# naturerobots/mesh_navigation

Hardware: AMD Instinct MI355X
Metric: plans/sec (Dijkstra makePlan device path incl. computeVectorMap, 1M-vertex mesh) (higher is better)
Workload: dtype f32

## Files before the change

### include/mnav.h

```cpp
#ifndef MNAV_H
#define MNAV_H

#include <stdint.h>

#ifdef __cplusplus
extern "C" {
#endif

#define MNAV_SUCCESS 0u
#define MNAV_CANCELED 51u
#define MNAV_INVALID_START 52u
#define MNAV_INVALID_GOAL 53u
#define MNAV_NO_PATH_FOUND 54u
#define MNAV_INTERNAL_ERROR 60u
#define MNAV_NONE 0xFFFFFFFFu

typedef struct mnav_ctx mnav_ctx;

typedef struct mnav_stats {
  uint32_t steps;
  uint32_t launches;
  uint32_t bands;
  uint32_t armed;
  float goal_dist;
// ... 309 lines not shown
uint64_t mnav_device_bytes(const mnav_ctx* ctx);

int mnav_shard_begin(mnav_ctx* ctx, uint32_t seed_vertex, uint32_t target_vertex, double goal_dist_offset, double cost_limit);
int mnav_shard_set_goal_tie(mnav_ctx* ctx, uint32_t tie_id);
int mnav_shard_rounds(mnav_ctx* ctx, uint32_t rounds, float* iface_buf_dev);
int mnav_shard_apply(mnav_ctx* ctx, const float* iface_buf_dev, float* local_min_out, float* target_dist_out);
int mnav_shard_finalize(mnav_ctx* ctx, float* dist_buf_dev, uint32_t* pred_buf_dev);
int mnav_shard_rounds_async(mnav_ctx* ctx, uint32_t rounds, float* iface_buf_dev, void* caller_stream);
int mnav_shard_apply_async(mnav_ctx* ctx, const float* iface_buf_dev, float* ctl_dev, void* caller_stream);

void mnav_cancel(mnav_ctx* ctx);

int mnav_get_stats(const mnav_ctx* ctx, mnav_stats* out);
int mnav_get_timing(const mnav_ctx* ctx, mnav_stats* out);
int mnav_tb_finalize_stats(mnav_ctx* ctx, uint64_t* skipped_pairs, uint64_t* reset_pairs, uint32_t* filled_at_start);
int mnav_set_band_width(mnav_ctx* ctx, float delta);
int mnav_set_dijkstra_engine(mnav_ctx* ctx, int engine);
int mnav_set_option(mnav_ctx* ctx, const char* name, double value);
double mnav_get_option(const mnav_ctx* ctx, const char* name);
int mnav_set_resident_outputs(mnav_ctx* ctx, int on);
int mnav_download_output(mnav_ctx* ctx, uint32_t slot, int what, void* host_out);
int mnav_vector_at(mnav_ctx* ctx, uint32_t slot, const uint32_t vs[3], const float bary[3], float out[3]);
int mnav_backtrack_cvp_batch(mnav_ctx* ctx, uint32_t n, const float* seed_pos, const uint32_t* seed_faces, const float* target_pos,
                             const uint32_t* target_faces, double step_width, int32_t inflation_layer, uint32_t cap,
                             float* positions_out, uint32_t* faces_out, uint32_t* n_out, int32_t* status_out);
int mnav_backtrack_cvp(mnav_ctx* ctx, const float seed_pos[3], uint32_t seed_face, const float target_pos[3], uint32_t target_face,
                       double step_width, int32_t inflation_layer, uint32_t cap, float* positions_out, uint32_t* faces_out,
                       uint32_t* n_out);
const void* mnav_device_output(const mnav_ctx* ctx, uint32_t slot, int what);
uint64_t mnav_algorithmic_bytes(const mnav_ctx* ctx);
// ... 7 lines not shown
```

### mesh_navigation_amd/capi.py

```python
from __future__ import annotations

import ctypes as C
import os
import sys
import time
import weakref
from dataclasses import dataclass

import numpy as np

from . import build as _build

NONE = 0xFFFFFFFF
SUCCESS, CANCELED, INVALID_START, INVALID_GOAL, NO_PATH_FOUND, INTERNAL_ERROR = 0, 51, 52, 53, 54, 60
SCHEDULE_NONE, SCHEDULE_COMMITTED, SCHEDULE_NO_SLOT, SCHEDULE_OPEN = 0, 1, 2, 3
SCHEDULE_SEED_FREE = 1
BEYOND_FIELD = 70
WALK_NO_FACE = -3

SYMBOLS = [
    "mnav_create", "mnav_destroy", "mnav_last_error", "mnav_set_face_circulation", "mnav_upload_mesh", "mnav_upload_costs",
    "mnav_compute_edge_weights", "mnav_combine_costs", "mnav_plan_dijkstra", "mnav_plan_cvp", "mnav_plan_dijkstra_batch", "mnav_plan_cvp_batch",
    "mnav_cancel", "mnav_get_stats", "mnav_get_timing", "mnav_tb_finalize_stats", "mnav_set_band_width", "mnav_set_dijkstra_engine", "mnav_device_output",
    "mnav_algorithmic_bytes", "mnav_shard_setup", "mnav_shard_setup_partition", "mnav_shard_walk", "mnav_device_bytes", "mnav_shard_info", "mnav_shard_begin", "mnav_shard_rounds", "mnav_shard_apply", "mnav_shard_rounds_async", "mnav_shard_apply_async",
    "mnav_shard_finalize", "mnav_update_costs", "mnav_update_edge_weights", "mnav_download_costs", "mnav_set_resident_outputs", "mnav_download_output",
    "mnav_vector_at", "mnav_backtrack_cvp", "mnav_backtrack_cvp_batch", "mnav_layer_upload", "mnav_layer_steepness", "mnav_layer_inflation", "mnav_layer_download",
    "mnav_combine_layers", "mnav_layer_stats", "mnav_layer_download_vectors", "mnav_combine_layers_update",
    "mnav_layer_obstacle", "mnav_obstacle_stats",
    "mnav_layer_height_diff", "mnav_layer_roughness", "mnav_layer_ridge", "mnav_neighbourhood_stats",
    "mnav_layer_border", "mnav_layer_clearance", "mnav_clearance_download", "mnav_clearance_stats",
    "mnav_locate", "mnav_locate_stats", "mnav_plan_dijkstra_batch_at", "mnav_plan_cvp_batch_at",
    "mnav_follow_batch", "mnav_follow_stats", "mnav_follow_rollout", "mnav_rollout_stats", "mnav_fleet_rollout", "mnav_fleet_rollout_stats",
    "mnav_fleet_rollout_yield", "mnav_fleet_yield_stats", "mnav_fleet_rollout_rings", "mnav_fleet_ring_stats",
    "mnav_map_configure", "mnav_map_compute", "mnav_map_layer_changed", "mnav_map_update_layer", "mnav_map_obstacle", "mnav_map_stats",
    "mnav_replan_dijkstra_batch", "mnav_replan_plans", "mnav_replan_stats", "mnav_replan_dijkstra_each", "mnav_replan_each_stats",
    "mnav_replan_warm_stats",
    "mnav_fleet_paths", "mnav_fleet_walks", "mnav_fleet_stats",
    "mnav_upload_face_normals", "mnav_fleet_plans", "mnav_fleet_walk_plans",
# ... 247 lines not shown
    L.mnav_replan_each_stats.argtypes = ([vp] + [C.POINTER(u32)] * 3 + [vp, vp, vp] + [C.POINTER(C.c_uint64)] * 2 + [C.POINTER(u32)] * 2
                                         + [C.POINTER(C.c_int32), vp])
    L.mnav_replan_warm_stats.restype = C.c_int
    L.mnav_replan_warm_stats.argtypes = [vp] + [C.POINTER(u32)] * 3 + [C.POINTER(C.c_uint64)] * 2 + [vp] + [C.POINTER(u32)] * 2
    L.mnav_replan_plans.restype = u32
    L.mnav_replan_plans.argtypes = [vp]
    L.mnav_replan_stats.restype = C.c_int
    L.mnav_replan_stats.argtypes = [vp, C.POINTER(u32), C.POINTER(u32), vp] + [C.POINTER(C.c_uint64)] * 2 + [C.POINTER(u32)] * 2 + [C.POINTER(C.c_float)] * 4
    L.mnav_cancel.argtypes = [vp]
    L.mnav_get_stats.restype = C.c_int
    L.mnav_get_stats.argtypes = [vp, C.POINTER(Stats)]
    L.mnav_get_timing.restype = C.c_int
    L.mnav_get_timing.argtypes = [vp, C.POINTER(Stats)]
    L.mnav_tb_finalize_stats.restype = C.c_int
    L.mnav_tb_finalize_stats.argtypes = [vp, C.POINTER(C.c_uint64), C.POINTER(C.c_uint64), C.POINTER(u32)]
    L.mnav_set_band_width.restype = C.c_int
    L.mnav_set_band_width.argtypes = [vp, C.c_float]
    L.mnav_set_dijkstra_engine.restype = C.c_int
    L.mnav_set_dijkstra_engine.argtypes = [vp, C.c_int]
    L.mnav_shard_set_goal_tie.restype = C.c_int
    L.mnav_shard_set_goal_tie.argtypes = [vp, u32]
    L.mnav_set_option.restype = C.c_int
    L.mnav_set_option.argtypes = [vp, C.c_char_p, C.c_double]
    L.mnav_get_option.restype = C.c_double
    L.mnav_get_option.argtypes = [vp, C.c_char_p]
    L.mnav_device_output.restype = vp
    L.mnav_device_output.argtypes = [vp, u32, C.c_int]
    L.mnav_set_resident_outputs.restype = C.c_int
    L.mnav_set_resident_outputs.argtypes = [vp, C.c_int]
    L.mnav_download_output.restype = C.c_int
# ... 563 lines not shown
            raise RuntimeError(f"mnav_shard_finalize failed ({rc}): {self._err()}")

    def stats(self) -> dict:
        s = Stats()
        self._L.mnav_get_stats(self._h, C.byref(s))
        d = s.as_dict()
        d["algorithmic_bytes"] = int(self._L.mnav_algorithmic_bytes(self._h))
        return d

    def tb_finalize_stats(self) -> dict:
        sk, rs, fl = C.c_uint64(0), C.c_uint64(0), C.c_uint32(0)
        if self._L.mnav_tb_finalize_stats(self._h, C.byref(sk), C.byref(rs), C.byref(fl)) != 0:
            raise RuntimeError(f"mnav_tb_finalize_stats failed: {self._err()}")
        return dict(skipped_pairs=int(sk.value), reset_pairs=int(rs.value), filled_at_start=bool(fl.value))

    def last_engine(self) -> str:
        e = int(self._L.mnav_last_engine(self._h))
        if e >= 256:
            ran = (["k_tile_round (tile rounds)"] if e & 128 else []) + ([_warm_name(1 if e & 1024 else 0)] if e & 512 else [])
            ran += [_engine_name(e & 127)] if (e & 127) != 127 else []
            return " + ".join(ran) if ran else "none (every plan kept)"
        if e in (5, 21) and self.replan_warm_stats()["live"]:
            return _warm_name(1 if e == 21 else 0)
        return _engine_name(e)

    def timing(self) -> dict:
        s = Stats()
        self._L.mnav_get_timing(self._h, C.byref(s))
        return s.as_dict()

# ... 648 lines not shown
```

### mesh_navigation_amd/csrc/mnav.hip

```cpp
#include <hip/hip_runtime.h>

#include <algorithm>
#include <array>
#include <atomic>
#include <chrono>
#include <cmath>
#include <cstdio>
#include <cstdlib>
#include <cstring>
#include <functional>
#include <map>
#include <string>
#include <vector>
#include <unordered_map>
#include <unistd.h>

#include "../../include/mnav.h"
#include "mnav_buf.h"
#include "mnav_build.h"
#include "mnav_eval.h"
#include "mnav_options.h"
#include "mnav_resident.h"

using namespace mnav;
// ... 1732 lines not shown
    if (hipSetDevice(ctx->device) != hipSuccess) { ctx->err = "hipSetDevice failed"; return -1; }
    const uint32_t nblk = (S.fin_np + 63u) / 64u;
    HIPCHK(hipMemsetAsync(S.fin_cnt, 0, 16, ctx->stream));
    hipLaunchKernelGGL(k_tb_fin_count, dim3(std::min<uint32_t>(((size_t)S.ntiles * nblk + kBlock - 1) / kBlock, 1024u)), dim3(kBlock), 0, ctx->stream,
                       S.umap.get(), S.uskip.get(), S.ntiles, nblk, S.umap_stride, S.fin_cnt.get());
    HIPCHK(hipGetLastError());
    HIPCHK(hipMemcpyAsync(cnt, S.fin_cnt, 16, hipMemcpyDeviceToHost, ctx->stream));
    HIPCHK(hipStreamSynchronize(ctx->stream));
  }
  if (skipped_pairs) *skipped_pairs = cnt[1];
  if (reset_pairs) *reset_pairs = (S.fin_stats && S.fin_reset) ? (uint64_t)S.ntiles * S.fin_np - cnt[0] : 0u;
  if (filled_at_start) *filled_at_start = S.filled_at_start ? 1u : 0u;
  return 0;
}

int mnav_get_timing(const mnav_ctx* ctx, mnav_stats* out)
{
  if (!ctx || !out) return -1;
  *out = ctx->stats;
  if (ctx->tb.count_pending) out->settled = 0;
  return 0;
}

int mnav_set_band_width(mnav_ctx* ctx, float delta)
{
  if (!ctx) return -1;
  ctx->delta_user = delta > 0.f ? delta : 0.f;
  return 0;
}

// ... 237 lines not shown
```

### mesh_navigation_amd/csrc/mnav_options.h

```cpp
#pragma once

#define MNAV_OPTION_LIST(X)                                                                                                              \
  X(verbose)                                                              \
  X(trace)                                                                                       \
  X(no_graph)             \
  X(debug_chunk)          \
  X(dijkstra_engine)                                 \
  X(blocks_per_plan)                                                                                 \
  X(tile_blocks)                                                                                    \
  X(cvp_wide)                                        \
  X(wide_waves)                                                                                      \
  X(cvp_groups)                          \
  X(max_steps) X(max_wall_s)                                                                                                             \
  X(cvp_verify)                                                                     \
  X(key_walk_max) X(descend_walk_max)                                                               \
  X(tile_size)                                                                                   \
  X(lazy_paths)                                                                                      \
  X(tile_band) X(rounds_band_mult)                                                                                                       \
  X(tb_tile)                                                       \
  X(tb_no_prefill) X(tb_band_mult) X(tb_waves_per_cu)                                                                                    \
  X(tb_kernel)            \
  X(tb_sched_lds)         \
  X(tb_fin_keep)          \
  X(tb_fin_cnt8)          \
  X(async_wg_per_cu) X(async_wg_per_plan) X(async_max_s)                                                                          \
  X(async_band_mult)                              \
  X(async_max_batch)                                           \
  X(async_ring_cap)             \
  X(nbhd_lds_cap)         \
  X(replan_log_cap)                                          \
  X(replan_fresh_below)   \
  X(replan_each_fresh_share)  \
  X(replan_repair_engine)  \
  X(replan_warm_min_plans)  \
  X(fleet_scratch_mb)     \
  X(dispatch_max_mb)      \
  X(dispatch_max_rounds)  \
// ... 52 lines not shown
```

### mesh_navigation_amd/csrc/mnav_tb.h

```cpp
#pragma once

#include "mnav_tb_build.h"

namespace {

namespace tb {

#define MNAV_CONST __attribute__((address_space(4)))
typedef uint32_t u32x16 __attribute__((ext_vector_type(16)));
typedef const MNAV_CONST u32x16* cblk8_t;
typedef __attribute__((address_space(3))) uint32_t* lds_u32_t;
enum { kTwSoff = 0, kTwSl = 1, kTwNv = 2, kTwNh = 3, kTwSweepOff = 4, kTwSweepChunks = 5, kTwPreOff = 6, kTwPreChunks = 7,
       kTwPostOff = 8, kTwPostChunks = 9, kTwExpOff = 10, kTwExpN = 11 };
static_assert(offsetof(TbTile, exp_n) == 4 * kTwExpN && offsetof(TbTile, sweep_off) == 4 * kTwSweepOff, "TbTile layout");

struct Ctl {
  uint32_t n_cand[2];
  uint32_t n_items, next_item;
  uint32_t err;
  uint32_t iters;
  unsigned long long acts;
  unsigned long long sweeps;
  unsigned long long items;
  unsigned long long wakes;
// ... 1 lines not shown

struct Args {
  const TbTile* tiles; const uint32_t* stream; const TbExp* exps;
  float* D; uint32_t* pend; uint32_t NP, ntiles;
  uint16_t* bucket; uint32_t* bcnt; uint2* items; Ctl* ctl;
  uint32_t* marr[2];
  uint32_t* mcarry;
  float* thr; float* bnd;
  const uint32_t* seed; const uint32_t* target;
  const uint2* vaddr; const uint32_t* vert_tile;
  double offset; float band;
  uint8_t* pflag; uint32_t nblk;
  unsigned long long* wstat; uint32_t wstat_slots;
  uint32_t item_plans;
  uint32_t sched_lds, min_copies;
};

__device__ __forceinline__ size_t slot_addr(const uint2 va, uint32_t NP, uint32_t p)
{
  return (size_t)va.x * NP + (size_t)p * (va.y >> 8) + (va.y & 255u);
}

__device__ __forceinline__ uint32_t ldsr(uint32_t off) { return *(lds_u32_t)(uintptr_t)off; }
__device__ __forceinline__ void ldsw(uint32_t off, uint32_t v) { *(lds_u32_t)(uintptr_t)off = v; }
typedef __attribute__((address_space(3))) u32x4* lds_u32x4_t;
__device__ __forceinline__ u32x4 ldsr4(uint32_t off) { return *(lds_u32x4_t)(uintptr_t)off; }

__device__ __forceinline__ uint32_t rfl(uint32_t x) { return (uint32_t)__builtin_amdgcn_readfirstlane((int)x); }

}
// ... 802 lines not shown
```

### mesh_navigation_amd/csrc/mnav_tb_host.h

```cpp
#pragma once

void tb_free_batch(mnav_ctx* ctx)
{
  TbState& S = ctx->tb;
  if (S.fill_stream) (void)hipStreamSynchronize(S.fill_stream);
  static_cast<TbBatch&>(S) = TbBatch{};
  S.count_pending = false; ctx->tb_args_valid = false;
  ctx->res.batch_state_freed();
}

void tb_free(mnav_ctx* ctx)
{
  tb_free_batch(ctx);
  static_cast<TbTables&>(ctx->tb) = TbTables{};
}

int tb_build(mnav_ctx* ctx)
{
  TbState& S = ctx->tb;
  if (S.built) return 0;
  if (opt_set(ctx->opt.tb_tile)) S.T = opt_u32(ctx->opt.tb_tile, S.T);
  if (S.T != 64 && S.T != 96 && S.T != 120 && S.T != 128) S.T = 120;
  HostTopology t;
  t.V = ctx->V; t.E = ctx->E; t.F = ctx->F;
// ... 254 lines not shown
  HIPCHK(hipMemsetAsync(ctx->d_mismatch, 0, 4, ctx->stream));
  if (!ctx->lazy_paths && tb_fields_upload(ctx, n, in, offset)) return -1;
  tb::Args A{};
  A.tiles = S.d_tiles; A.stream = S.d_stream; A.exps = S.d_exps; A.D = S.D; A.pend = S.pend; A.pflag = S.pflag; A.nblk = (n + 63u) / 64u; A.NP = n; A.ntiles = S.ntiles;
  A.bucket = S.bucket; A.bcnt = S.bcnt; A.items = S.items; A.ctl = S.ctl; A.wstat = S.wstat; A.wstat_slots = kTbStatSlots;
  A.marr[0] = S.marr[0]; A.marr[1] = S.marr[1]; A.mcarry = S.mcarry;
  A.thr = S.thr; A.bnd = S.bnd; A.seed = S.seed; A.target = S.target; A.vaddr = S.d_vaddr; A.vert_tile = S.d_vert_tile;
  A.offset = offset;
  const bool v_fits = S.T == 120 && S.max_nh <= kTbvGhostRows;
  const double density = (double)n / std::sqrt((double)std::max(S.ntiles, 1u));
  S.kernel = (v_fits && density >= 8.0) ? 1 : 0;
  if (opt_set(ctx->opt.tb_kernel)) S.kernel = (opt_u32(ctx->opt.tb_kernel, 0u) == 1u && v_fits) ? 1 : 0;
  A.item_plans = S.kernel == 1 ? 64u : kTbItemPlans;
  A.sched_lds = (tb_sched_lds_fits(n) && !(opt_set(ctx->opt.tb_sched_lds) && !opt_on(ctx->opt.tb_sched_lds))) ? 1u : 0u;
  A.min_copies = A.sched_lds ? kTbMinCopiesLds : kTbMinCopies;
  {
    const float band_mult = (S.kernel == 1 && density < 40.0) ? 4.0f : S.band_mult;
    float band = (ctx->delta_auto / 3.0f) * std::sqrt((float)S.T) * band_mult;
    if (opt_set(ctx->opt.tb_band_mult)) band = (ctx->delta_auto / 3.0f) * std::sqrt((float)S.T) * (float)ctx->opt.tb_band_mult;
    if (ctx->tile_band_user > 0.f) band = ctx->tile_band_user;
    A.band = band;
  }
  HIPCHK(hipEventRecord(ctx->ev[1], ctx->stream));
  if (!warm) {
    bool prefilled = was_clean >= n;
    if (!prefilled) {
      if (S.D2 && S.d2_clean && S.d2_clean_np >= n) {
        std::swap(S.D, S.D2); A.D = S.D;
        HIPCHK(hipStreamWaitEvent(ctx->stream, S.fill_done, 0));
        prefilled = true;
// ... 97 lines not shown
```

### mesh_navigation_amd/csrc/mnav_tbv.h

```cpp
#pragma once

#pragma clang diagnostic push
#pragma clang diagnostic ignored "-Winline-asm"
namespace {
namespace tbv {

#define TBV_COMPILER_VGPRS __attribute__((amdgpu_num_vgpr(20)))
constexpr int kRows = 120;
constexpr int kGhostRows = (int)kTbvGhostRows;
static_assert(kGhostRows == 64, "the window starts at v72: ghosts v[72:135], owned rows v[136:255]");

template <int R> __device__ __forceinline__ void img_set(uint32_t x) { asm volatile("v_mov_b32 v[136+%c1], %0" : : "v"(x), "n"(R)); }
template <int R> __device__ __forceinline__ uint32_t img_get() { uint32_t x; asm volatile("v_mov_b32 %0, v[136+%c1]" : "=v"(x) : "n"(R)); return x; }
template <int R> __device__ __forceinline__ void img_load(const uint32_t* p) { asm volatile("global_load_dword v[136+%c1], %0, off" : : "v"(p), "n"(R) : "memory"); }
template <int C> __device__ __forceinline__ void img_load_quad(const void* p) { asm volatile("global_load_dwordx4 v[136+%c1:139+%c1], %0, off offset:%c2" : : "v"(p), "n"(4 * C), "n"(16 * C) : "memory"); }
template <int Q> __device__ __forceinline__ void ghost_load_quad(const void* p) { asm volatile("global_load_dwordx4 v[72+%c1:75+%c1], %0, off offset:%c2" : : "v"(p), "n"(4 * Q), "n"(16 * (kRows / 4 + Q)) : "memory"); }
template <int C> __device__ __forceinline__ void img_store_quad(void* p) { asm volatile("global_store_dwordx4 %0, v[136+%c1:139+%c1], off offset:%c2" : : "v"(p), "n"(4 * C), "n"(16 * C) : "memory"); }
__device__ __forceinline__ void img_loads_wait() { asm volatile("s_waitcnt vmcnt(0)" : : : "memory"); }
template <int I, int N, class F> __device__ __forceinline__ void static_for(F&& f)
{
  if constexpr (I < N) { f(std::integral_constant<int, I>{}); static_for<I + 1, N>(f); }
}
__device__ __forceinline__ uint32_t win_read(uint32_t row)
{
// ... 39 lines not shown
  "s_cbranch_scc0 Ltbv_pc" #tag "_%=\n\t"                                                                              \
  "v_cndmask_b32 v68, v67, v62, vcc\n\t"                                                                               \
  "v_min_u32 v65, v65, v68\n\t"                                                                                        \
  "v_mov_b32 v66, v67\n\t"                                                                                             \
  "s_bitcmp1_b32 s[" #i3 "], 17\n\t"                                                                                   \
  "s_cbranch_scc0 Ltbv_pn" #tag "_%=\n\t"                                                                              \
  "s_or_b32 m0, s85, 0x8000\n\t"                                                                                       \
  "v_mov_b32 v72, v65\n\t"                                                                                             \
  "s_mov_b32 m0, 0\n\t"                                                                                                \
  "v_mov_b32 v65, v67\n\t"                                                                                             \
  "s_add_u32 s85, s85, 1\n\t"                                                                                          \
  "s_branch Ltbv_pn" #tag "_%=\n\t"                                                                                    \
  "Ltbv_pc" #tag "_%=:\n\t"                                                                                            \
  "v_mov_b32 v66, v62\n\t"                                                                                             \
  "Ltbv_pn" #tag "_%=:\n\t"
#define TBV_LOAD(b)                                                                                                    \
  "s_add_u32 s86, s72, s68\n\t"  "s_addc_u32 s87, s73, 0\n\t"                                                          \
  "global_load_dwordx4 v[" #b ":" #b "+3], v64, s[86:87]\n\t"                                                          \
  "s_add_u32 s68, s68, 0x100\n\t"  "s_cmp_eq_u32 s68, s75\n\t"  "s_cselect_b32 s68, 0, s68\n\t"
#define TBV_SLOAD(S)                                                                                                   \
  "s_load_dwordx16 s[" #S ":" #S "+15], s[72:73], s78\n\t"                                                             \
  "s_add_u32 s78, s78, 0x100\n\t"  "s_cmp_eq_u32 s78, s75\n\t"  "s_cselect_b32 s78, 0, s78\n\t"
#define TBV_CHUNK(BLOCK, b, SA, SB, tag, END)                                                                          \
  "s_waitcnt vmcnt(3) lgkmcnt(0)\n\t"                                                                                  \
  TBV_SLOAD(SB)                                                                                                        \
  "s_set_gpr_idx_on s74, gpr_idx(SRC1)\n\t"                                                                            \
  BLOCK(b, SA, SA + 4, SA + 8, SA + 12, tag##0)  BLOCK(b + 1, SA + 1, SA + 5, SA + 9, SA + 13, tag##1)                 \
  BLOCK(b + 2, SA + 2, SA + 6, SA + 10, SA + 14, tag##2)  BLOCK(b + 3, SA + 3, SA + 7, SA + 11, SA + 15, tag##3)       \
  "s_set_gpr_idx_off\n\t"                                                                                              \
  TBV_LOAD(b)                                                                                                          \
  "s_sub_u32 s80, s80, 1\n\t"                                                                                          \
  "s_cmp_lg_u32 s80, 0\n\t"                                                                                            \
  "s_cbranch_scc1 Ltbv_nx" #tag "_%=\n\t"                                                                              \
  END                                                                                                                  \
  "Ltbv_nx" #tag "_%=:\n\t"
#define TBV_END_SWEEP                                                                                                  \
  "s_mov_b32 s80, s74\n\t"                                                                                             \
  "s_add_u32 s84, s84, 1\n\t"                                                                                          \
  "s_or_b64 s[88:89], s[88:89], s[70:71]\n\t"                                                                          \
  "s_or_b64 s[70:71], s[70:71], s[82:83]\n\t"                                                                          \
  "s_cmp_eq_u64 s[70:71], 0\n\t"                                                                                       \
  "s_cbranch_scc1 Ltbv_done_%=\n\t"                                                                                    \
  "s_cmp_ge_u32 s84, s81\n\t"                                                                                          \
  "s_cbranch_scc1 Ltbv_over_%=\n\t"                                                                                    \
  "s_mov_b64 s[70:71], 0\n\t"
#define TBV_END_PASS "s_branch Ltbv_done_%=\n\t"
#define TBV_LOOP(BLOCK, END)                                                                                           \
  TBV_LOAD(40) TBV_LOAD(44) TBV_LOAD(48) TBV_LOAD(52)                                                                  \
  TBV_SLOAD(36)                                                                                                        \
  "Ltbv_top_%=:\n\t"                                                                                                   \
  TBV_CHUNK(BLOCK, 40, 36, 52, c0, END) TBV_CHUNK(BLOCK, 44, 52, 36, c1, END) TBV_CHUNK(BLOCK, 48, 36, 52, c2, END) TBV_CHUNK(BLOCK, 52, 52, 36, c3, END) \
  "s_branch Ltbv_top_%=\n\t"
#define TBV_CLOBBERS "memory", "vcc", "scc", "m0", "s36", "s37", "s38", "s39", "s40", "s41", "s42", "s43", "s44", "s45", "s46", "s47", "s48", "s49", "s50", "s51", \
  "s52", "s53", "s54", "s55", "s56", "s57", "s58", "s59", "s60", "s61", "s62", "s63", "s64", "s65", "s66", "s67", "s68", "s70", "s71", "s72", "s73", "s74", "s75", \
  "s78", "s80", "s81", "s82", "s83", "s84", "s85", "s86", "s87", "s88", "s89", "v40", "v68", "v255"

struct Uni { uint32_t lo, hi, nch; };
__device__ __forceinline__ Uni uni(const uint32_t* first, uint32_t nch)
{
  const unsigned long long a = (unsigned long long)(uintptr_t)first;
  return Uni{ tb::rfl((uint32_t)a), tb::rfl((uint32_t)(a >> 32)), tb::rfl(nch) };
}

__device__ __forceinline__ uint32_t tbv_sweeps(const uint32_t* sweep0, uint32_t nch, uint32_t first_order, uint32_t cap, uint32_t lane_off,
                                               uint32_t force, bool& overrun, unsigned long long& lowered)
{
  uint32_t sweeps, ovr, low_lo, low_hi;
  const Uni u = uni(sweep0, nch);
  first_order = tb::rfl(first_order); cap = tb::rfl(cap); force = tb::rfl(force);
  asm volatile(
      "v_mov_b32 v64, %[off]\n\t"
      "s_mov_b32 s72, %[stlo]\n\t"
      "s_mov_b32 s73, %[sthi]\n\t"
      "s_mov_b32 s74, %[nch]\n\t"
      "s_lshl_b32 s75, s74, 10\n\t"
      "s_mov_b32 s81, %[cap]\n\t"
      "s_mov_b32 s82, %[force]\n\t"
      "s_mov_b32 s83, %[force]\n\t"
      "s_lshl_b32 s68, s74, 8\n\t"
      "s_mul_i32 s68, s68, %[ord]\n\t"
      "s_mov_b32 s78, s68\n\t"
      "s_mov_b32 s80, s74\n\t"
      "s_mov_b32 s84, 0\n\t"
      "s_mov_b64 s[70:71], 0\n\t"
      "s_mov_b64 s[88:89], 0\n\t"
      TBV_LOOP(TBV_BLOCK_SWEEP, TBV_END_SWEEP)
      "Ltbv_over_%=:\n\t"
      "s_mov_b32 %[ovr], 1\n\t"
      "s_branch Ltbv_end_%=\n\t"
      "Ltbv_done_%=:\n\t"
      "s_mov_b32 %[ovr], 0\n\t"
      "Ltbv_end_%=:\n\t"
      "s_mov_b32 %[sw], s84\n\t"
      "s_mov_b32 %[llo], s88\n\t"
      "s_mov_b32 %[lhi], s89\n\t"
      "s_waitcnt vmcnt(0) lgkmcnt(0)\n\t"
      : [sw] "=s"(sweeps), [ovr] "=s"(ovr), [llo] "=s"(low_lo), [lhi] "=s"(low_hi)
      : [stlo] "s"(u.lo), [sthi] "s"(u.hi), [nch] "s"(u.nch), [ord] "s"(first_order), [cap] "s"(cap), [off] "v"(lane_off), [force] "s"(force)
      : TBV_CLOBBERS);
  overrun = ovr != 0u;
  lowered = ((unsigned long long)low_hi << 32) | low_lo;
  return sweeps;
}

__device__ __forceinline__ void tbv_pre(const uint32_t* pre0, uint32_t nch, uint32_t lane_off, uint32_t& min_new, uint32_t& order)
{
  const Uni u = uni(pre0, nch);
  asm volatile(
      "v_mov_b32 v64, %[off]\n\t"
      "v_mov_b32 v67, 0x7f800000\n\t"
      "v_mov_b32 v65, v67\n\t"
      "v_mov_b32 v66, 0\n\t"
      "s_mov_b32 s72, %[stlo]\n\t"
      "s_mov_b32 s73, %[sthi]\n\t"
      "s_mov_b32 s74, %[nch]\n\t"
      "s_lshl_b32 s75, s74, 8\n\t"
      "s_mov_b32 s68, 0\n\t"
      "s_mov_b32 s78, 0\n\t"
      "s_mov_b32 s80, s74\n\t"
      TBV_LOOP(TBV_BLOCK_PRE, TBV_END_PASS)
      "Ltbv_done_%=:\n\t"
      "v_mov_b32 %[mn], v65\n\t"
      "v_mov_b32 %[od], v66\n\t"
      "s_waitcnt vmcnt(0) lgkmcnt(0)\n\t"
      : [mn] "=v"(min_new), [od] "=v"(order)
      : [stlo] "s"(u.lo), [sthi] "s"(u.hi), [nch] "s"(u.nch), [off] "v"(lane_off)
      : TBV_CLOBBERS);
}

__device__ __forceinline__ void tbv_post(const uint32_t* post0, uint32_t nch, uint32_t lane_off)
{
  const Uni u = uni(post0, nch);
  asm volatile(
      "v_mov_b32 v64, %[off]\n\t"
      "v_mov_b32 v67, 0x7f800000\n\t"
      "v_mov_b32 v65, v67\n\t"
      "v_mov_b32 v66, v67\n\t"
      "s_mov_b32 s85, 0\n\t"
      "s_mov_b32 s72, %[stlo]\n\t"
      "s_mov_b32 s73, %[sthi]\n\t"
      "s_mov_b32 s74, %[nch]\n\t"
      "s_lshl_b32 s75, s74, 8\n\t"
      "s_mov_b32 s68, 0\n\t"
      "s_mov_b32 s78, 0\n\t"
      "s_mov_b32 s80, s74\n\t"
      TBV_LOOP(TBV_BLOCK_POST, TBV_END_PASS)
      "Ltbv_done_%=:\n\t"
      "s_waitcnt vmcnt(0) lgkmcnt(0)\n\t"
      :
      : [stlo] "s"(u.lo), [sthi] "s"(u.hi), [nch] "s"(u.nch), [off] "v"(lane_off)
      : TBV_CLOBBERS);
}

typedef float f32x4u __attribute__((ext_vector_type(4), aligned(4)));
typedef float f32x2u __attribute__((ext_vector_type(2), aligned(4)));
typedef const MNAV_CONST uint32_t* cwords_t;
template <class P> __device__ __forceinline__ cwords_t cwords(P* p) { return (cwords_t)(uintptr_t)p; }

}
// ... 27 lines not shown
    const uint32_t p = A.bucket[(size_t)t * NP + start + min((uint32_t)lane, max(count, 1u) - 1u)];
    MNAV_GLOBAL float* const sl = as_global(A.D) + ((size_t)soff * NP + (size_t)p * slen);
    TB_STAMP(0);
    tbv::static_for<0, T / 4>([&](auto c) { tbv::img_load_quad<decltype(c)::value>((const void*)sl); });
    {
      const uint32_t nq = (nh + 3u) >> 2;
      tbv::static_for<0, tbv::kGhostRows / 4>([&](auto q) { if ((uint32_t)decltype(q)::value < nq) tbv::ghost_load_quad<decltype(q)::value>((const void*)sl); });
    }
    uint32_t it_n = 0;
    if (lane == 0) it_n = atomicAdd(&A.ctl->next_item, 1u);
    tbv::img_loads_wait();
    it_n = gridDim.x + tb::rfl(it_n);
    u32x2 item_n = { 0u, 0u };
    if (it_n < n_items) item_n = ((MNAV_GLOBAL const u32x2*)as_global(A.items))[it_n];
    TB_STAMP(1);
    uint32_t first_order = 0;
    bool changed = false;
    if (pre_chunks) {
      uint32_t mn, gord;
      tbv::tbv_pre(vstream + (size_t)pre_off * kTbChunk, pre_chunks, lane_off, mn, gord);
      changed = mn != kTbInfBits;
      const bool votes = active && changed;
      uint32_t bestc = 0;
#pragma unroll
      for (uint32_t o = 0; o < 4; ++o) {
        const uint32_t cn = (uint32_t)__popcll(__ballot(votes && (gord & 3u) == o));
        if (cn > bestc) { bestc = cn; first_order = o; }
      }
    }
    TB_STAMP(2);
    uint32_t sweep = 1;
    if (sweep_chunks) {
      bool overrun;
      unsigned long long lowered;
      sweep = tbv::tbv_sweeps(vstream + (size_t)sweep_off * kTbChunk, sweep_chunks, first_order, 16u * T, lane_off, 0u, overrun, lowered);
      if (overrun && lane == 0) A.ctl->err = 1u;
      changed = changed || ((lowered >> lane) & 1ull);
    }
    my_sweeps += sweep;
    TB_STAMP(3);
    if (post_chunks) {
      tbv::tbv_post(vstream + (size_t)post_off * kTbChunk, post_chunks, lane_off);
      TB_STAMP(7);
      MNAV_GLOBAL uint32_t* const pend_p = as_global(A.pend) + p;
      MNAV_GLOBAL uint8_t* const pflag_p = as_global(A.pflag) + (p >> 6);
      uint32_t n_first = 0, mbest = kTbInfBits;
      for (uint32_t g0 = 0; g0 < grp_n; g0 += 4u) {
        uint32_t best[4], old[4];
        bool want[4];
#pragma unroll
// ... 46 lines not shown
    TB_STAMP(6);
    it = it_n; item = item_n;
  }
#ifdef MNAV_TB_TIMING
  if (lane == 0) for (int k = 0; k < 8; ++k) if (tt[k]) atomicAdd(&g_tb_timing[k], tt[k]);
#endif
  my_wakes = wave_sum(my_wakes); my_acts = wave_sum(my_acts);
  if (__any(my_first != 0u) && lane == 0) A.ctl->n_cand[par ^ 1] = 1u;
  if (lane == 0 && my_items && blockIdx.x < A.wstat_slots) {
    unsigned long long* const ws = A.wstat + 4u * blockIdx.x;
    ws[0] += (unsigned long long)my_items; ws[1] += (unsigned long long)my_acts; ws[2] += (unsigned long long)my_sweeps; ws[3] += (unsigned long long)my_wakes;
  }
}

__global__ __launch_bounds__(64) TBV_COMPILER_VGPRS
void k_tbv_micro(const uint32_t* __restrict__ stream, uint32_t nch, uint32_t first_order, uint32_t cap, uint32_t force, uint32_t reps,
                 uint32_t* __restrict__ img, uint32_t* __restrict__ out)
{
  const int lane = threadIdx.x;
  uint32_t* const my = img + (size_t)blockIdx.x * tbv::kRows * 64 + lane;
  tbv::static_for<0, tbv::kRows>([&](auto r) { constexpr int R = decltype(r)::value; tbv::img_load<R>(my + R * 64); });
  tbv::img_loads_wait();
  uint32_t total = 0, over = 0;
  for (uint32_t k = 0; k < reps; ++k) {
    bool ovr;
    unsigned long long low;
    total += tbv::tbv_sweeps(stream, nch, first_order, cap, 16u * ((uint32_t)lane & 15u), force ? ~0u : 0u, ovr, low);
    over |= ovr ? 1u : 0u;
  }
  tbv::static_for<0, tbv::kRows>([&](auto r) { constexpr int R = decltype(r)::value; my[R * 64] = tbv::img_get<R>(); });
  if (lane == 0) { out[2 * blockIdx.x] = total; out[2 * blockIdx.x + 1] = over; }
}

}

extern "C" int mnav_debug_tbv_sweeps(const uint32_t* stream_host, uint32_t nch, uint32_t first_order, uint32_t cap, uint32_t force, uint32_t reps,
                                     uint32_t waves, uint32_t* img_host, uint32_t* out_host, float* ms_out)
{
  DevBuf<uint32_t> d_s, d_i, d_o;
  const size_t ns = (size_t)4 * nch * 64 + 8 * 64, ni = (size_t)waves * tbv::kRows * 64;
  if (d_s.alloc(4 * ns) != hipSuccess || d_i.alloc(4 * ni) != hipSuccess || d_o.alloc(8 * (size_t)waves) != hipSuccess) return -1;
  (void)hipMemset(d_s, 0, 4 * ns);
  (void)hipMemcpy(d_s, stream_host, (size_t)4 * 4 * nch * 64, hipMemcpyHostToDevice);
  (void)hipMemcpy(d_i, img_host, 4 * ni, hipMemcpyHostToDevice);
  Event e0, e1;
  (void)hipEventCreate(e0.out()); (void)hipEventCreate(e1.out());
  (void)hipEventRecord(e0, 0);
  hipLaunchKernelGGL(k_tbv_micro, dim3(waves), dim3(64), 0, 0, d_s, nch, first_order, cap, force, reps, d_i, d_o);
  (void)hipEventRecord(e1, 0);
  const hipError_t e = hipDeviceSynchronize();
  float ms = 0.f;
  (void)hipEventElapsedTime(&ms, e0, e1);
  if (ms_out) *ms_out = ms;
  (void)hipMemcpy(img_host, d_i, 4 * ni, hipMemcpyDeviceToHost);
  (void)hipMemcpy(out_host, d_o, 8 * (size_t)waves, hipMemcpyDeviceToHost);
  return e == hipSuccess ? 0 : -2;
}
#pragma clang diagnostic pop
```

Baseline: 48040.

## Sweep TBV orientations in vote-ranked sequence instead of fixed rotation

Replaces the single best first-order choice with a 16-entry 2-bit sequence of sweep orientations built from the ballot counts of every orientation, ranked by vote. The asm sweep loop now walks stream chunks through per-orientation cursors, taking branches at segment ends in place of wrapping modulo the full stream. The goal is to converge the sweeps in fewer passes by visiting orientations in order of how many lanes improved along them. The cost is extra scalar cursor logic and branches in the hot asm loop plus more clobbered SGPRs. It also adds an option to fall back to rotation and a stats query API.

```diff
diff --git a/include/mnav.h b/include/mnav.h
--- a/include/mnav.h
+++ b/include/mnav.h
@@ -347,6 +347,7 @@
 int mnav_get_stats(const mnav_ctx* ctx, mnav_stats* out);
 int mnav_get_timing(const mnav_ctx* ctx, mnav_stats* out);
 int mnav_tb_finalize_stats(mnav_ctx* ctx, uint64_t* skipped_pairs, uint64_t* reset_pairs, uint32_t* filled_at_start);
+int mnav_tb_engine_stats(const mnav_ctx* ctx, uint32_t* iterations, uint64_t* items, uint64_t* activations, uint64_t* sweeps, uint64_t* wakes);
 int mnav_set_band_width(mnav_ctx* ctx, float delta);
 int mnav_set_dijkstra_engine(mnav_ctx* ctx, int engine);
 int mnav_set_option(mnav_ctx* ctx, const char* name, double value);
diff --git a/mesh_navigation_amd/capi.py b/mesh_navigation_amd/capi.py
--- a/mesh_navigation_amd/capi.py
+++ b/mesh_navigation_amd/capi.py
@@ -21,7 +21,7 @@
 SYMBOLS = [
     "mnav_create", "mnav_destroy", "mnav_last_error", "mnav_set_face_circulation", "mnav_upload_mesh", "mnav_upload_costs",
     "mnav_compute_edge_weights", "mnav_combine_costs", "mnav_plan_dijkstra", "mnav_plan_cvp", "mnav_plan_dijkstra_batch", "mnav_plan_cvp_batch",
-    "mnav_cancel", "mnav_get_stats", "mnav_get_timing", "mnav_tb_finalize_stats", "mnav_set_band_width", "mnav_set_dijkstra_engine", "mnav_device_output",
+    "mnav_cancel", "mnav_get_stats", "mnav_get_timing", "mnav_tb_finalize_stats", "mnav_tb_engine_stats", "mnav_set_band_width", "mnav_set_dijkstra_engine", "mnav_device_output",
     "mnav_algorithmic_bytes", "mnav_shard_setup", "mnav_shard_setup_partition", "mnav_shard_walk", "mnav_device_bytes", "mnav_shard_info", "mnav_shard_begin", "mnav_shard_rounds", "mnav_shard_apply", "mnav_shard_rounds_async", "mnav_shard_apply_async",
     "mnav_shard_finalize", "mnav_update_costs", "mnav_update_edge_weights", "mnav_download_costs", "mnav_set_resident_outputs", "mnav_download_output",
     "mnav_vector_at", "mnav_backtrack_cvp", "mnav_backtrack_cvp_batch", "mnav_layer_upload", "mnav_layer_steepness", "mnav_layer_inflation", "mnav_layer_download",
@@ -299,6 +299,8 @@
     L.mnav_get_timing.argtypes = [vp, C.POINTER(Stats)]
     L.mnav_tb_finalize_stats.restype = C.c_int
     L.mnav_tb_finalize_stats.argtypes = [vp, C.POINTER(C.c_uint64), C.POINTER(C.c_uint64), C.POINTER(u32)]
+    L.mnav_tb_engine_stats.restype = C.c_int
+    L.mnav_tb_engine_stats.argtypes = [vp, C.POINTER(u32)] + [C.POINTER(C.c_uint64)] * 4
     L.mnav_set_band_width.restype = C.c_int
     L.mnav_set_band_width.argtypes = [vp, C.c_float]
     L.mnav_set_dijkstra_engine.restype = C.c_int
@@ -892,6 +894,14 @@
             raise RuntimeError(f"mnav_tb_finalize_stats failed: {self._err()}")
         return dict(skipped_pairs=int(sk.value), reset_pairs=int(rs.value), filled_at_start=bool(fl.value))
 
+    def tb_engine_stats(self) -> dict:
+        it = C.c_uint32(0)
+        items, acts, sweeps, wakes = (C.c_uint64(0) for _ in range(4))
+        if self._L.mnav_tb_engine_stats(self._h, C.byref(it), C.byref(items), C.byref(acts), C.byref(sweeps), C.byref(wakes)) != 0:
+            raise RuntimeError(f"mnav_tb_engine_stats failed: {self._err()}")
+        return dict(iterations=int(it.value), items=int(items.value), activations=int(acts.value), sweeps=int(sweeps.value), wakes=int(wakes.value),
+                    sweeps_per_item=(sweeps.value / items.value) if items.value else 0.0)
+
     def last_engine(self) -> str:
         e = int(self._L.mnav_last_engine(self._h))
         if e >= 256:
diff --git a/mesh_navigation_amd/csrc/mnav.hip b/mesh_navigation_amd/csrc/mnav.hip
--- a/mesh_navigation_amd/csrc/mnav.hip
+++ b/mesh_navigation_amd/csrc/mnav.hip
@@ -1770,6 +1770,18 @@
   return 0;
 }
 
+int mnav_tb_engine_stats(const mnav_ctx* ctx, uint32_t* iterations, uint64_t* items, uint64_t* activations, uint64_t* sweeps, uint64_t* wakes)
+{
+  if (!ctx) return -1;
+  const tb::Ctl& K = ctx->tb.last;
+  if (iterations) *iterations = K.iters;
+  if (items) *items = K.items;
+  if (activations) *activations = K.acts;
+  if (sweeps) *sweeps = K.sweeps;
+  if (wakes) *wakes = K.wakes;
+  return 0;
+}
+
 int mnav_get_timing(const mnav_ctx* ctx, mnav_stats* out)
 {
   if (!ctx || !out) return -1;
diff --git a/mesh_navigation_amd/csrc/mnav_options.h b/mesh_navigation_amd/csrc/mnav_options.h
--- a/mesh_navigation_amd/csrc/mnav_options.h
+++ b/mesh_navigation_amd/csrc/mnav_options.h
@@ -21,6 +21,7 @@
   X(tb_no_prefill) X(tb_band_mult) X(tb_waves_per_cu)                                                                                    \
   X(tb_kernel)            \
   X(tb_sched_lds)         \
+  X(tb_sweep_seq)         \
   X(tb_fin_keep)          \
   X(tb_fin_cnt8)          \
   X(async_wg_per_cu) X(async_wg_per_plan) X(async_max_s)                                                                          \
diff --git a/mesh_navigation_amd/csrc/mnav_tb.h b/mesh_navigation_amd/csrc/mnav_tb.h
--- a/mesh_navigation_amd/csrc/mnav_tb.h
+++ b/mesh_navigation_amd/csrc/mnav_tb.h
@@ -39,6 +39,7 @@
   unsigned long long* wstat; uint32_t wstat_slots;
   uint32_t item_plans;
   uint32_t sched_lds, min_copies;
+  uint32_t sweep_seq;
 };
 
 __device__ __forceinline__ size_t slot_addr(const uint2 va, uint32_t NP, uint32_t p)
diff --git a/mesh_navigation_amd/csrc/mnav_tb_host.h b/mesh_navigation_amd/csrc/mnav_tb_host.h
--- a/mesh_navigation_amd/csrc/mnav_tb_host.h
+++ b/mesh_navigation_amd/csrc/mnav_tb_host.h
@@ -292,6 +292,7 @@
   A.item_plans = S.kernel == 1 ? 64u : kTbItemPlans;
   A.sched_lds = (tb_sched_lds_fits(n) && !(opt_set(ctx->opt.tb_sched_lds) && !opt_on(ctx->opt.tb_sched_lds))) ? 1u : 0u;
   A.min_copies = A.sched_lds ? kTbMinCopiesLds : kTbMinCopies;
+  A.sweep_seq = opt_u32(ctx->opt.tb_sweep_seq, 1u) != 0u ? 1u : 0u;
   {
     const float band_mult = (S.kernel == 1 && density < 40.0) ? 4.0f : S.band_mult;
     float band = (ctx->delta_auto / 3.0f) * std::sqrt((float)S.T) * band_mult;
diff --git a/mesh_navigation_amd/csrc/mnav_tbv.h b/mesh_navigation_amd/csrc/mnav_tbv.h
--- a/mesh_navigation_amd/csrc/mnav_tbv.h
+++ b/mesh_navigation_amd/csrc/mnav_tbv.h
@@ -1,4 +1,5 @@
 #pragma once
+#include "mnav_tbv_seq.h"
 
 #pragma clang diagnostic push
 #pragma clang diagnostic ignored "-Winline-asm"
@@ -77,21 +78,33 @@
   "Ltbv_pc" #tag "_%=:\n\t"                                                                                            \
   "v_mov_b32 v66, v62\n\t"                                                                                             \
   "Ltbv_pn" #tag "_%=:\n\t"
-#define TBV_LOAD(b)                                                                                                    \
+#define TBV_LOAD(b, tag)                                                                                               \
   "s_add_u32 s86, s72, s68\n\t"  "s_addc_u32 s87, s73, 0\n\t"                                                          \
   "global_load_dwordx4 v[" #b ":" #b "+3], v64, s[86:87]\n\t"                                                          \
-  "s_add_u32 s68, s68, 0x100\n\t"  "s_cmp_eq_u32 s68, s75\n\t"  "s_cselect_b32 s68, 0, s68\n\t"
-#define TBV_SLOAD(S)                                                                                                   \
+  "s_add_u32 s68, s68, 0x100\n\t"  "s_cmp_eq_u32 s68, s76\n\t"  "s_cbranch_scc1 Ltbv_vf" #tag "_%=\n\t"                \
+  "Ltbv_vr" #tag "_%=:\n\t"
+#define TBV_SLOAD(S, tag)                                                                                              \
   "s_load_dwordx16 s[" #S ":" #S "+15], s[72:73], s78\n\t"                                                             \
-  "s_add_u32 s78, s78, 0x100\n\t"  "s_cmp_eq_u32 s78, s75\n\t"  "s_cselect_b32 s78, 0, s78\n\t"
+  "s_add_u32 s78, s78, 0x100\n\t"  "s_cmp_eq_u32 s78, s77\n\t"  "s_cbranch_scc1 Ltbv_sf" #tag "_%=\n\t"                \
+  "Ltbv_sr" #tag "_%=:\n\t"
+#define TBV_CURSOR_NEXT(POS, END, IDX)                                                                                 \
+  "s_add_u32 " IDX ", " IDX ", 1\n\t"  "s_cmp_gt_u32 " IDX ", 15\n\t"  "s_cselect_b32 s86, 4, 0\n\t"  "s_sub_u32 " IDX ", " IDX ", s86\n\t" \
+  "s_lshl_b32 s86, " IDX ", 1\n\t"  "s_lshr_b32 s86, s69, s86\n\t"  "s_and_b32 s86, s86, 3\n\t"                        \
+  "s_mul_i32 " POS ", s86, s75\n\t"  "s_add_u32 " END ", " POS ", s75\n\t"
+#define TBV_LOAD_FIX(tag)  "Ltbv_vf" #tag "_%=:\n\t" TBV_CURSOR_NEXT("s68", "s76", "s79") "s_branch Ltbv_vr" #tag "_%=\n\t"
+#define TBV_SLOAD_FIX(tag) "Ltbv_sf" #tag "_%=:\n\t" TBV_CURSOR_NEXT("s78", "s77", "s90") "s_branch Ltbv_sr" #tag "_%=\n\t"
+#define TBV_CURSORS_INIT                                                                                               \
+  "s_lshl_b32 s75, s74, 8\n\t"                                                                                         \
+  "s_and_b32 s68, s69, 3\n\t"  "s_mul_i32 s68, s68, s75\n\t"  "s_add_u32 s76, s68, s75\n\t"  "s_mov_b32 s79, 0\n\t"      \
+  "s_mov_b32 s78, s68\n\t"  "s_mov_b32 s77, s76\n\t"  "s_mov_b32 s90, 0\n\t"
 #define TBV_CHUNK(BLOCK, b, SA, SB, tag, END)                                                                          \
   "s_waitcnt vmcnt(3) lgkmcnt(0)\n\t"                                                                                  \
-  TBV_SLOAD(SB)                                                                                                        \
+  TBV_SLOAD(SB, tag)                                                                                                   \
   "s_set_gpr_idx_on s74, gpr_idx(SRC1)\n\t"                                                                            \
   BLOCK(b, SA, SA + 4, SA + 8, SA + 12, tag##0)  BLOCK(b + 1, SA + 1, SA + 5, SA + 9, SA + 13, tag##1)                 \
   BLOCK(b + 2, SA + 2, SA + 6, SA + 10, SA + 14, tag##2)  BLOCK(b + 3, SA + 3, SA + 7, SA + 11, SA + 15, tag##3)       \
   "s_set_gpr_idx_off\n\t"                                                                                              \
-  TBV_LOAD(b)                                                                                                          \
+  TBV_LOAD(b, tag)                                                                                                     \
   "s_sub_u32 s80, s80, 1\n\t"                                                                                          \
   "s_cmp_lg_u32 s80, 0\n\t"                                                                                            \
   "s_cbranch_scc1 Ltbv_nx" #tag "_%=\n\t"                                                                              \
@@ -109,14 +122,17 @@
   "s_mov_b64 s[70:71], 0\n\t"
 #define TBV_END_PASS "s_branch Ltbv_done_%=\n\t"
 #define TBV_LOOP(BLOCK, END)                                                                                           \
-  TBV_LOAD(40) TBV_LOAD(44) TBV_LOAD(48) TBV_LOAD(52)                                                                  \
-  TBV_SLOAD(36)                                                                                                        \
+  TBV_LOAD(40, p0) TBV_LOAD(44, p1) TBV_LOAD(48, p2) TBV_LOAD(52, p3)                                                  \
+  TBV_SLOAD(36, p0)                                                                                                    \
   "Ltbv_top_%=:\n\t"                                                                                                   \
   TBV_CHUNK(BLOCK, 40, 36, 52, c0, END) TBV_CHUNK(BLOCK, 44, 52, 36, c1, END) TBV_CHUNK(BLOCK, 48, 36, 52, c2, END) TBV_CHUNK(BLOCK, 52, 52, 36, c3, END) \
-  "s_branch Ltbv_top_%=\n\t"
+  "s_branch Ltbv_top_%=\n\t"                                                                                          \
+  TBV_LOAD_FIX(p0) TBV_LOAD_FIX(p1) TBV_LOAD_FIX(p2) TBV_LOAD_FIX(p3) TBV_SLOAD_FIX(p0)                                \
+  TBV_LOAD_FIX(c0) TBV_LOAD_FIX(c1) TBV_LOAD_FIX(c2) TBV_LOAD_FIX(c3)                                                  \
+  TBV_SLOAD_FIX(c0) TBV_SLOAD_FIX(c1) TBV_SLOAD_FIX(c2) TBV_SLOAD_FIX(c3)
 #define TBV_CLOBBERS "memory", "vcc", "scc", "m0", "s36", "s37", "s38", "s39", "s40", "s41", "s42", "s43", "s44", "s45", "s46", "s47", "s48", "s49", "s50", "s51", \
-  "s52", "s53", "s54", "s55", "s56", "s57", "s58", "s59", "s60", "s61", "s62", "s63", "s64", "s65", "s66", "s67", "s68", "s70", "s71", "s72", "s73", "s74", "s75", \
-  "s78", "s80", "s81", "s82", "s83", "s84", "s85", "s86", "s87", "s88", "s89", "v40", "v68", "v255"
+  "s52", "s53", "s54", "s55", "s56", "s57", "s58", "s59", "s60", "s61", "s62", "s63", "s64", "s65", "s66", "s67", "s68", "s69", "s70", "s71", "s72", "s73", "s74", "s75", \
+  "s76", "s77", "s78", "s79", "s80", "s81", "s82", "s83", "s84", "s85", "s86", "s87", "s88", "s89", "s90", "v40", "v68", "v255"
 
 struct Uni { uint32_t lo, hi, nch; };
 __device__ __forceinline__ Uni uni(const uint32_t* first, uint32_t nch)
@@ -125,24 +141,22 @@
   return Uni{ tb::rfl((uint32_t)a), tb::rfl((uint32_t)(a >> 32)), tb::rfl(nch) };
 }
 
-__device__ __forceinline__ uint32_t tbv_sweeps(const uint32_t* sweep0, uint32_t nch, uint32_t first_order, uint32_t cap, uint32_t lane_off,
+__device__ __forceinline__ uint32_t tbv_sweeps(const uint32_t* sweep0, uint32_t nch, uint32_t seq, uint32_t cap, uint32_t lane_off,
                                                uint32_t force, bool& overrun, unsigned long long& lowered)
 {
   uint32_t sweeps, ovr, low_lo, low_hi;
   const Uni u = uni(sweep0, nch);
-  first_order = tb::rfl(first_order); cap = tb::rfl(cap); force = tb::rfl(force);
+  seq = tb::rfl(seq); cap = tb::rfl(cap); force = tb::rfl(force);
   asm volatile(
       "v_mov_b32 v64, %[off]\n\t"
       "s_mov_b32 s72, %[stlo]\n\t"
       "s_mov_b32 s73, %[sthi]\n\t"
       "s_mov_b32 s74, %[nch]\n\t"
-      "s_lshl_b32 s75, s74, 10\n\t"
+      "s_mov_b32 s69, %[seq]\n\t"
+      TBV_CURSORS_INIT
       "s_mov_b32 s81, %[cap]\n\t"
       "s_mov_b32 s82, %[force]\n\t"
       "s_mov_b32 s83, %[force]\n\t"
-      "s_lshl_b32 s68, s74, 8\n\t"
-      "s_mul_i32 s68, s68, %[ord]\n\t"
-      "s_mov_b32 s78, s68\n\t"
       "s_mov_b32 s80, s74\n\t"
       "s_mov_b32 s84, 0\n\t"
       "s_mov_b64 s[70:71], 0\n\t"
@@ -159,7 +173,7 @@
       "s_mov_b32 %[lhi], s89\n\t"
       "s_waitcnt vmcnt(0) lgkmcnt(0)\n\t"
       : [sw] "=s"(sweeps), [ovr] "=s"(ovr), [llo] "=s"(low_lo), [lhi] "=s"(low_hi)
-      : [stlo] "s"(u.lo), [sthi] "s"(u.hi), [nch] "s"(u.nch), [ord] "s"(first_order), [cap] "s"(cap), [off] "v"(lane_off), [force] "s"(force)
+      : [stlo] "s"(u.lo), [sthi] "s"(u.hi), [nch] "s"(u.nch), [seq] "s"(seq), [cap] "s"(cap), [off] "v"(lane_off), [force] "s"(force)
       : TBV_CLOBBERS);
   overrun = ovr != 0u;
   lowered = ((unsigned long long)low_hi << 32) | low_lo;
@@ -177,9 +191,8 @@
       "s_mov_b32 s72, %[stlo]\n\t"
       "s_mov_b32 s73, %[sthi]\n\t"
       "s_mov_b32 s74, %[nch]\n\t"
-      "s_lshl_b32 s75, s74, 8\n\t"
-      "s_mov_b32 s68, 0\n\t"
-      "s_mov_b32 s78, 0\n\t"
+      "s_mov_b32 s69, 0\n\t"
+      TBV_CURSORS_INIT
       "s_mov_b32 s80, s74\n\t"
       TBV_LOOP(TBV_BLOCK_PRE, TBV_END_PASS)
       "Ltbv_done_%=:\n\t"
@@ -203,9 +216,8 @@
       "s_mov_b32 s72, %[stlo]\n\t"
       "s_mov_b32 s73, %[sthi]\n\t"
       "s_mov_b32 s74, %[nch]\n\t"
-      "s_lshl_b32 s75, s74, 8\n\t"
-      "s_mov_b32 s68, 0\n\t"
-      "s_mov_b32 s78, 0\n\t"
+      "s_mov_b32 s69, 0\n\t"
+      TBV_CURSORS_INIT
       "s_mov_b32 s80, s74\n\t"
       TBV_LOOP(TBV_BLOCK_POST, TBV_END_PASS)
       "Ltbv_done_%=:\n\t"
@@ -263,26 +275,25 @@
     u32x2 item_n = { 0u, 0u };
     if (it_n < n_items) item_n = ((MNAV_GLOBAL const u32x2*)as_global(A.items))[it_n];
     TB_STAMP(1);
-    uint32_t first_order = 0;
+    uint32_t seq = tbv_seq::tbv_seq_rotation(0u);
     bool changed = false;
     if (pre_chunks) {
       uint32_t mn, gord;
       tbv::tbv_pre(vstream + (size_t)pre_off * kTbChunk, pre_chunks, lane_off, mn, gord);
       changed = mn != kTbInfBits;
       const bool votes = active && changed;
-      uint32_t bestc = 0;
+      uint32_t cn[4];
 #pragma unroll
-      for (uint32_t o = 0; o < 4; ++o) {
-        const uint32_t cn = (uint32_t)__popcll(__ballot(votes && (gord & 3u) == o));
-        if (cn > bestc) { bestc = cn; first_order = o; }
-      }
+      for (uint32_t o = 0; o < 4; ++o) cn[o] = (uint32_t)__popcll(__ballot(votes && (gord & 3u) == o));
+      seq = tbv_seq::tbv_seq_build(cn[0], cn[1], cn[2], cn[3]);
+      if (!A.sweep_seq) seq = tbv_seq::tbv_seq_rotation(seq & 3u);
     }
     TB_STAMP(2);
     uint32_t sweep = 1;
     if (sweep_chunks) {
       bool overrun;
       unsigned long long lowered;
-      sweep = tbv::tbv_sweeps(vstream + (size_t)sweep_off * kTbChunk, sweep_chunks, first_order, 16u * T, lane_off, 0u, overrun, lowered);
+      sweep = tbv::tbv_sweeps(vstream + (size_t)sweep_off * kTbChunk, sweep_chunks, seq, 16u * T, lane_off, 0u, overrun, lowered);
       if (overrun && lane == 0) A.ctl->err = 1u;
       changed = changed || ((lowered >> lane) & 1ull);
     }
@@ -359,7 +370,7 @@
 }
 
 __global__ __launch_bounds__(64) TBV_COMPILER_VGPRS
-void k_tbv_micro(const uint32_t* __restrict__ stream, uint32_t nch, uint32_t first_order, uint32_t cap, uint32_t force, uint32_t reps,
+void k_tbv_micro(const uint32_t* __restrict__ stream, uint32_t nch, uint32_t seq, uint32_t cap, uint32_t force, uint32_t reps,
                  uint32_t* __restrict__ img, uint32_t* __restrict__ out)
 {
   const int lane = threadIdx.x;
@@ -370,7 +381,7 @@
   for (uint32_t k = 0; k < reps; ++k) {
     bool ovr;
     unsigned long long low;
-    total += tbv::tbv_sweeps(stream, nch, first_order, cap, 16u * ((uint32_t)lane & 15u), force ? ~0u : 0u, ovr, low);
+    total += tbv::tbv_sweeps(stream, nch, seq, cap, 16u * ((uint32_t)lane & 15u), force ? ~0u : 0u, ovr, low);
     over |= ovr ? 1u : 0u;
   }
   tbv::static_for<0, tbv::kRows>([&](auto r) { constexpr int R = decltype(r)::value; my[R * 64] = tbv::img_get<R>(); });
@@ -379,9 +390,10 @@
 
 }
 
-extern "C" int mnav_debug_tbv_sweeps(const uint32_t* stream_host, uint32_t nch, uint32_t first_order, uint32_t cap, uint32_t force, uint32_t reps,
-                                     uint32_t waves, uint32_t* img_host, uint32_t* out_host, float* ms_out)
-{
+extern "C" int mnav_debug_tbv_sweeps_seq(const uint32_t* stream_host, uint32_t nch, uint32_t seq, uint32_t cap, uint32_t force, uint32_t reps,
+                                         uint32_t waves, uint32_t* img_host, uint32_t* out_host, float* ms_out)
+{
+  if (nch < 1u || !waves) return -1;
   DevBuf<uint32_t> d_s, d_i, d_o;
   const size_t ns = (size_t)4 * nch * 64 + 8 * 64, ni = (size_t)waves * tbv::kRows * 64;
   if (d_s.alloc(4 * ns) != hipSuccess || d_i.alloc(4 * ni) != hipSuccess || d_o.alloc(8 * (size_t)waves) != hipSuccess) return -1;
@@ -391,7 +403,7 @@
   Event e0, e1;
   (void)hipEventCreate(e0.out()); (void)hipEventCreate(e1.out());
   (void)hipEventRecord(e0, 0);
-  hipLaunchKernelGGL(k_tbv_micro, dim3(waves), dim3(64), 0, 0, d_s, nch, first_order, cap, force, reps, d_i, d_o);
+  hipLaunchKernelGGL(k_tbv_micro, dim3(waves), dim3(64), 0, 0, d_s, nch, seq, cap, force, reps, d_i, d_o);
   (void)hipEventRecord(e1, 0);
   const hipError_t e = hipDeviceSynchronize();
   float ms = 0.f;
@@ -401,4 +413,10 @@
   (void)hipMemcpy(out_host, d_o, 8 * (size_t)waves, hipMemcpyDeviceToHost);
   return e == hipSuccess ? 0 : -2;
 }
+
+extern "C" int mnav_debug_tbv_sweeps(const uint32_t* stream_host, uint32_t nch, uint32_t first_order, uint32_t cap, uint32_t force, uint32_t reps,
+                                     uint32_t waves, uint32_t* img_host, uint32_t* out_host, float* ms_out)
+{
+  return mnav_debug_tbv_sweeps_seq(stream_host, nch, tbv_seq::tbv_seq_rotation(first_order), cap, force, reps, waves, img_host, out_host, ms_out);
+}
 #pragma clang diagnostic pop
diff --git a/mesh_navigation_amd/csrc/mnav_tbv_seq.h b/mesh_navigation_amd/csrc/mnav_tbv_seq.h
--- /dev/null
+++ b/mesh_navigation_amd/csrc/mnav_tbv_seq.h
@@ -0,0 +1,33 @@
+#pragma once
+#include <stdint.h>
+
+#if defined(__HIPCC__) || defined(__CUDACC__)
+#define MNAV_SEQ_HD __host__ __device__ inline
+#else
+#define MNAV_SEQ_HD inline
+#endif
+
+namespace tbv_seq {
+
+constexpr uint32_t kEntries = 16;
+
+MNAV_SEQ_HD uint32_t tbv_seq_next_index(uint32_t k) { return k + 1u > 15u ? k + 1u - 4u : k + 1u; }
+MNAV_SEQ_HD uint32_t tbv_seq_index(uint32_t k) { return k < kEntries ? k : 12u + (k & 3u); }
+MNAV_SEQ_HD uint32_t tbv_seq_at(uint32_t seq, uint32_t k) { return (seq >> (2u * tbv_seq_index(k))) & 3u; }
+
+MNAV_SEQ_HD uint32_t tbv_seq_rotation(uint32_t first) { return (uint32_t)(0xE4E4E4E4E4E4E4E4ull >> (2u * (first & 3u))); }
+
+MNAV_SEQ_HD uint32_t tbv_seq_build(uint32_t c0, uint32_t c1, uint32_t c2, uint32_t c3)
+{
+  uint32_t k0 = (c0 << 2) | 3u, k1 = (c1 << 2) | 2u, k2 = (c2 << 2) | 1u, k3 = c3 << 2;
+  const uint32_t n = (c0 != 0u) + (c1 != 0u) + (c2 != 0u) + (c3 != 0u);
+#define MNAV_SEQ_CX(a, b) { const uint32_t hi = a > b ? a : b, lo = a > b ? b : a; a = hi; b = lo; }
+  MNAV_SEQ_CX(k0, k1) MNAV_SEQ_CX(k2, k3) MNAV_SEQ_CX(k0, k2) MNAV_SEQ_CX(k1, k3) MNAV_SEQ_CX(k1, k2)
+#undef MNAV_SEQ_CX
+  const uint32_t all = (~k0 & 3u) | (~k1 & 3u) << 2 | (~k2 & 3u) << 4 | (~k3 & 3u) << 6;
+  const uint32_t prefix = all & ((1u << (2u * n)) - 1u);
+  const uint32_t next = n ? ((all >> (2u * n - 2u)) + 1u) & 3u : 0u;
+  return prefix | tbv_seq_rotation(next) << (2u * n);
+}
+
+}
```

Result: no change. 48820 (median of 6 runs) (+1.6%).
